# NVlabs/FoundationPose

Hardware: NVIDIA H100
Metric: pose-hypotheses/sec at 640x480 RGB-D, 252 hyp, 5 refine iters (higher is better)
Workload: dtype f16

## Files before the change

foundationpose_b200/csrc/fp_common.cuh:

```cuda
#pragma once
#include <cuda.h>
#include <cuda_fp16.h>
#include <cuda_runtime.h>
#include <stdint.h>
#include <stdio.h>
#include <string.h>

#include <atomic>

namespace fp {

void note_launches(int n);
unsigned long long launch_count();
void set_capturing(bool on);
inline bool device_bit_test(const std::atomic<unsigned long long>& m) {
  int d = 0;
  cudaGetDevice(&d);
  return (m.load(std::memory_order_acquire) >> (d & 63)) & 1ull;
}
inline void device_bit_set(std::atomic<unsigned long long>& m) {
  int d = 0;
  cudaGetDevice(&d);
  m.fetch_or(1ull << (d & 63), std::memory_order_release);
}
int num_sms();

void set_last_error(const char* fmt, ...);
int check_device_ptr(const void* p, const char* what, const char* fn = "fp_pose_errors");
#define FP_CUDA_OK(expr)                                                                   \
  do {                                                                                     \
    cudaError_t _e = (expr);                                                               \
    if (_e != cudaSuccess) {                                                               \
      fp::set_last_error("%s:%d: %s -> %s", __FILE__, __LINE__, #expr, cudaGetErrorString(_e)); \
      return -2;                                                                           \
    }                                                                                      \
  } while (0)
#define FP_REQUIRE(cond, ...)                                                              \
  do {                                                                                     \
    if (!(cond)) {                                                                         \
      fp::set_last_error(__VA_ARGS__);                                                     \
      return -1;                                                                           \
    }                                                                                      \
  } while (0)
#define FP_TRY(expr)     \
  do {                   \
    int _rc = (expr);    \
    if (_rc) return _rc; \
  } while (0)

bool pdl_enabled();
void pdl_skip_next();

template <typename... KArgs, typename... Args>
inline cudaError_t launch_pdl(void (*kernel)(KArgs...), dim3 grid, dim3 block, size_t smem, cudaStream_t stream,
                              int cluster_x, Args... args) {
  cudaLaunchConfig_t cfg;
  memset(&cfg, 0, sizeof(cfg));
  cfg.gridDim = grid;
  cfg.blockDim = block;
  cfg.dynamicSmemBytes = smem;
  cfg.stream = stream;
  cudaLaunchAttribute attr[2];
  int na = 0;
  if (cluster_x > 1) {
    attr[na].id = cudaLaunchAttributeClusterDimension;
    attr[na].val.clusterDim.x = cluster_x;
    attr[na].val.clusterDim.y = 1;
    attr[na].val.clusterDim.z = 1;
    ++na;
  }
  if (pdl_enabled()) {
    attr[na].id = cudaLaunchAttributeProgrammaticStreamSerialization;
    attr[na].val.programmaticStreamSerializationAllowed = 1;
    ++na;
  }
  cfg.attrs = attr;
  cfg.numAttrs = na;
  return cudaLaunchKernelEx(&cfg, kernel, KArgs(args)...);
}

__device__ __forceinline__ void pdl_wait() { asm volatile("griddepcontrol.wait;" ::: "memory"); }
__device__ __forceinline__ void pdl_trigger() { asm volatile("griddepcontrol.launch_dependents;" ::: "memory"); }

__device__ __forceinline__ uint32_t smem_u32(const void* p) {
  return static_cast<uint32_t>(__cvta_generic_to_shared(p));
}

__device__ __forceinline__ void mbar_init(uint64_t* bar, uint32_t count) {
  asm volatile("mbarrier.init.shared::cta.b64 [%0], %1;" ::"r"(smem_u32(bar)), "r"(count));
}
__device__ __forceinline__ void mbar_fence_init() {
  asm volatile("fence.mbarrier_init.release.cluster;" ::: "memory");
}
__device__ __forceinline__ void mbar_expect_tx(uint64_t* bar, uint32_t bytes) {
  asm volatile("mbarrier.arrive.expect_tx.shared::cta.b64 _, [%0], %1;" ::"r"(smem_u32(bar)),
               "r"(bytes)
               : "memory");
}
__device__ __forceinline__ void mbar_arrive(uint64_t* bar) {
  asm volatile("mbarrier.arrive.shared::cta.b64 _, [%0];" ::"r"(smem_u32(bar)) : "memory");
}
__device__ __forceinline__ void mbar_wait(uint64_t* bar, uint32_t parity) {
  asm volatile(
      "{\n\t"
      ".reg .pred P1;\n\t"
      "WAIT_%=:\n\t"
      "mbarrier.try_wait.parity.shared::cta.b64 P1, [%0], %1, %2;\n\t"
      "@P1 bra DONE_%=;\n\t"
      "bra WAIT_%=;\n\t"
      "DONE_%=:\n\t"
      "}" ::"r"(smem_u32(bar)),
      "r"(parity), "r"(0x989680)
      : "memory");
}

__device__ __forceinline__ void tma_load_5d(const CUtensorMap* map, uint64_t* bar, void* dst,
                                            int c0, int c1, int c2, int c3, int c4) {
  asm volatile(
      "cp.async.bulk.tensor.5d.shared::cluster.global.mbarrier::complete_tx::bytes"
      " [%0], [%1, {%3, %4, %5, %6, %7}], [%2];" ::"r"(smem_u32(dst)),
      "l"(reinterpret_cast<uint64_t>(map)), "r"(smem_u32(bar)), "r"(c0), "r"(c1), "r"(c2),
      "r"(c3), "r"(c4)
      : "memory");
}
__device__ __forceinline__ void tma_load_2d(const CUtensorMap* map, uint64_t* bar, void* dst,
                                            int c0, int c1) {
  asm volatile(
      "cp.async.bulk.tensor.2d.shared::cluster.global.mbarrier::complete_tx::bytes"
      " [%0], [%1, {%3, %4}], [%2];" ::"r"(smem_u32(dst)),
      "l"(reinterpret_cast<uint64_t>(map)), "r"(smem_u32(bar)), "r"(c0), "r"(c1)
      : "memory");
}
__device__ __forceinline__ void tma_store_5d(const CUtensorMap* map, const void* src, int c0, int c1, int c2, int c3,
                                             int c4) {
  asm volatile("cp.async.bulk.tensor.5d.global.shared::cta.bulk_group [%0, {%2, %3, %4, %5, %6}], [%1];" ::"l"(
                   reinterpret_cast<uint64_t>(map)),
               "r"(smem_u32(src)), "r"(c0), "r"(c1), "r"(c2), "r"(c3), "r"(c4)
               : "memory");
}
__device__ __forceinline__ void tma_prefetch_desc(const CUtensorMap* map) {
  asm volatile("prefetch.tensormap [%0];" ::"l"(reinterpret_cast<uint64_t>(map)) : "memory");
}

__device__ __forceinline__ uint32_t cluster_nctarank() {
  uint32_t r;
  asm volatile("mov.u32 %0, %%cluster_nctarank;" : "=r"(r));
  return r;
}
__device__ __forceinline__ uint32_t cluster_ctarank() {
  uint32_t r;
  asm volatile("mov.u32 %0, %%cluster_ctarank;" : "=r"(r));
  return r;
}
__device__ __forceinline__ void cluster_sync_all() {
  asm volatile("barrier.cluster.arrive.release.aligned;" ::: "memory");
  asm volatile("barrier.cluster.wait.acquire.aligned;" ::: "memory");
}

template <uint32_t N>
__device__ __forceinline__ void regs_release() {
  asm volatile("setmaxnreg.dec.sync.aligned.u32 %0;" ::"n"(N));
}
template <uint32_t N>
__device__ __forceinline__ void regs_acquire() {
  asm volatile("setmaxnreg.inc.sync.aligned.u32 %0;" ::"n"(N));
}

__device__ __forceinline__ void wgmma_fence() { asm volatile("wgmma.fence.sync.aligned;" ::: "memory"); }
__device__ __forceinline__ void wgmma_commit() { asm volatile("wgmma.commit_group.sync.aligned;" ::: "memory"); }
template <int N>
__device__ __forceinline__ void wgmma_wait() {
  asm volatile("wgmma.wait_group.sync.aligned %0;" ::"n"(N) : "memory");
}
template <int N>
__device__ __forceinline__ void fence_regs(float (&d)[N]) {
#pragma unroll
  for (int i = 0; i < N; ++i) asm volatile("" : "+f"(d[i])::"memory");
}

__device__ __forceinline__ uint64_t gmma_desc_sw128(uint32_t smem_addr, uint32_t sbo = 1024) {
  uint64_t d = 0;
  d |= (uint64_t)((smem_addr & 0x3FFFF) >> 4);
  d |= (uint64_t)1 << 16;
  d |= (uint64_t)(sbo >> 4) << 32;
  d |= (uint64_t)1 << 62;
  return d;
}
__device__ __forceinline__ uint64_t gmma_desc_mn_sw128(uint32_t smem_addr, uint32_t lbo) {
  uint64_t d = 0;
  d |= (uint64_t)((smem_addr & 0x3FFFF) >> 4);
  d |= (uint64_t)((lbo >> 4) & 0x3FFF) << 16;
  d |= (uint64_t)(1024 >> 4) << 32;
  d |= (uint64_t)1 << 62;
  return d;
}
__device__ __forceinline__ uint64_t gmma_desc_linear(uint32_t smem_addr, uint32_t lbo, uint32_t sbo) {
  uint64_t d = 0;
  d |= (uint64_t)((smem_addr & 0x3FFFF) >> 4);
  d |= (uint64_t)(lbo >> 4) << 16;
  d |= (uint64_t)(sbo >> 4) << 32;
  return d;
}

__device__ __forceinline__ void ldsm_x4_trans(uint32_t addr, uint32_t (&r)[4]) {
  asm volatile("ldmatrix.sync.aligned.m8n8.x4.trans.shared.b16 {%0, %1, %2, %3}, [%4];"
               : "=r"(r[0]), "=r"(r[1]), "=r"(r[2]), "=r"(r[3])
               : "r"(addr)
               : "memory");
}
__device__ __forceinline__ void stsm_x4_trans(uint32_t addr, const uint32_t (&r)[4]) {
  asm volatile("stmatrix.sync.aligned.m8n8.x4.trans.shared.b16 [%0], {%1, %2, %3, %4};" ::"r"(addr), "r"(r[0]),
               "r"(r[1]), "r"(r[2]), "r"(r[3])
               : "memory");
}

__device__ __forceinline__ uint32_t pack_half2(float a, float b) {
  __half2 h = __floats2half2_rn(a, b);
  return *reinterpret_cast<uint32_t*>(&h);
}

}
```

foundationpose_b200/csrc/fp_linear.cu:

```cuda
#include <stdlib.h>
#include <string.h>

#include "fp_common.cuh"
#include "fp_gemm.cuh"
#include "fp_wgmma.cuh"

namespace fp {

int encode_map_f16(CUtensorMap* map, const void* base, int rank, const uint64_t* dims, const uint64_t* strides_bytes,
                   const uint32_t* box);

constexpr int kLwsK = 512;
constexpr int kLwsKBlocks = kLwsK / 64;
constexpr int kLwsRows = 64;
constexpr int kLwsCols = 128;
constexpr int kLwsThreads = 384;
constexpr int kLwsBoxBytes = kLwsCols * 64 * 2;
constexpr int kLwsPanelBytes = kLwsKBlocks * kLwsBoxBytes;
constexpr int kLwsStages = kLwsKBlocks;
constexpr int kLwsStageBytes = kLwsRows * 64 * 2;
constexpr int kLwsSlabBytes = kLwsRows * 64 * 2;
constexpr int kLwsSlabs = 4;
constexpr int kLwsSmemBytes =
    kLwsPanelBytes + kLwsStages * kLwsStageBytes + kLwsSlabs * kLwsSlabBytes + 1024  + 256 ;
static_assert(kLwsSmemBytes <= 232448, "the weight-stationary linear kernel exceeds the 227 KB opt-in shared memory");
static_assert((2 * kLwsStages + 4) * 8 <= 256, "the mbarriers must fit their 256 bytes");

constexpr uint32_t kOrderBar = 2;
constexpr uint32_t kWgBar = 4;

struct LinearWsParams {
  int row_tiles;
  int total;
  const float* bias;
  int has_res;
  int relu;
};

__device__ __forceinline__ void named_sync(uint32_t id, uint32_t count) {
  asm volatile("bar.sync %0, %1;" ::"r"(id), "r"(count) : "memory");
}
__device__ __forceinline__ void named_arrive(uint32_t id, uint32_t count) {
  asm volatile("bar.arrive %0, %1;" ::"r"(id), "r"(count) : "memory");
}

__global__ void __launch_bounds__(kLwsThreads, 1)
    linear_ws_kernel(const __grid_constant__ CUtensorMap map_a, const __grid_constant__ CUtensorMap map_w,
                     const __grid_constant__ CUtensorMap map_out, const __grid_constant__ CUtensorMap map_res,
                     const __grid_constant__ LinearWsParams p) {
  extern __shared__ uint8_t smem_raw[];
  uint8_t* smem = smem_raw + ((1024u - (smem_u32(smem_raw) & 1023u)) & 1023u);
  uint8_t* panel = smem;
  uint8_t* ring = panel + kLwsPanelBytes;
  uint8_t* staging = ring + kLwsStages * kLwsStageBytes;
  uint64_t* bars = reinterpret_cast<uint64_t*>(staging + kLwsSlabs * kLwsSlabBytes);
  uint64_t* full = bars;
  uint64_t* empty = bars + kLwsStages;
  uint64_t* panel_full = bars + 2 * kLwsStages;
  uint64_t* panel_empty = panel_full + 1;
  uint64_t* res_full = panel_full + 2;

  const int i0 = (int)((long long)blockIdx.x * p.total / gridDim.x);
  const int n = (int)((long long)(blockIdx.x + 1) * p.total / gridDim.x) - i0;
  const int panel0 = i0 / p.row_tiles;
  const int jb = min(n, (panel0 + 1) * p.row_tiles - i0);
  const bool reload = jb < n;

  if (threadIdx.x == 0) {
    tma_prefetch_desc(&map_a);
    tma_prefetch_desc(&map_w);
    tma_prefetch_desc(&map_out);
    if (p.has_res) tma_prefetch_desc(&map_res);
    for (int s = 0; s < kLwsStages; ++s) {
      mbar_init(&full[s], 1);
      mbar_init(&empty[s], 128);
    }
    mbar_init(panel_full, 1);
    mbar_init(panel_empty, 256);
    mbar_init(&res_full[0], 1);
    mbar_init(&res_full[1], 1);
    mbar_fence_init();
    mbar_expect_tx(panel_full, kLwsPanelBytes);
    for (int kb = 0; kb < kLwsKBlocks; ++kb)
      tma_load_2d(&map_w, panel_full, panel + kb * kLwsBoxBytes, kb * 64, panel0 * kLwsCols);
  }
  __syncthreads();
  pdl_trigger();
  pdl_wait();

  if (threadIdx.x < 128) {
    if (threadIdx.x == 0) {
      for (int j = 0; j < n; ++j) {
        if (j == jb) {
          mbar_wait(panel_empty, 0);
          mbar_expect_tx(panel_full, kLwsPanelBytes);
          for (int kb = 0; kb < kLwsKBlocks; ++kb)
            tma_load_2d(&map_w, panel_full, panel + kb * kLwsBoxBytes, kb * 64, (panel0 + 1) * kLwsCols);
        }
        const int row0 = ((i0 + j) % p.row_tiles) * kLwsRows;
        for (int kb = 0; kb < kLwsKBlocks; ++kb) {
          mbar_wait(&empty[kb], (uint32_t)((j & 1) ^ 1));
          mbar_expect_tx(&full[kb], kLwsStageBytes);
          tma_load_2d(&map_a, &full[kb], ring + kb * kLwsStageBytes, kb * 64, row0);
        }
      }
    }
    return;
  }

  const int ct = threadIdx.x - 128;
  const int w = ct >> 7;
  const int lane = threadIdx.x & 31;
  const int r0 = 16 * ((ct >> 5) & 3) + (lane >> 2);
  const int cq = 2 * (lane & 3);
  const bool leader = (ct & 127) == 0;
  uint8_t* slabs = staging + w * 2 * kLwsSlabBytes;
  if (reload && w >= jb) mbar_arrive(panel_empty);
  float acc[64];
#pragma unroll
  for (int i = 0; i < 64; ++i) acc[i] = 0.f;
  for (int j = w, it = 0; j < n; j += 2, ++it) {
    const int item = i0 + j;
    const int pn = item / p.row_tiles;
    const int row0 = (item - pn * p.row_tiles) * kLwsRows;
    if (j > 0) named_sync(kOrderBar + w, 256);
    mbar_wait(panel_full, j >= jb ? 1u : 0u);
    for (int kb = 0; kb < kLwsKBlocks; ++kb) {
      mbar_wait(&full[kb], (uint32_t)(j & 1));
      const uint64_t da = gmma_desc_sw128(smem_u32(ring + kb * kLwsStageBytes));
      const uint64_t db = gmma_desc_sw128(smem_u32(panel + kb * kLwsBoxBytes));
      wgmma_fence();
#pragma unroll
      for (int k = 0; k < 4; ++k)
        Wgmma<128>::ss(acc, da + (uint64_t)(2 * k), db + (uint64_t)(2 * k), (kb > 0 || k > 0) ? 1u : 0u);
      wgmma_commit();
      if (kb == 0 && leader) {
        asm volatile("cp.async.bulk.wait_group.read 0;" ::: "memory");
        if (p.has_res) {
          mbar_expect_tx(&res_full[w], 2 * kLwsSlabBytes);
          for (int s = 0; s < 2; ++s)
            tma_load_5d(&map_res, &res_full[w], slabs + s * kLwsSlabBytes, pn * kLwsCols + 64 * s, row0, 0, 0, 0);
        }
      }
      if (kb > 0) {
        wgmma_wait<1>();
        mbar_arrive(&empty[kb - 1]);
      }
    }
    if (j + 1 < n) named_arrive(kOrderBar + (w ^ 1), 256);
    wgmma_wait<0>();
    fence_regs(acc);
    mbar_arrive(&empty[kLwsKBlocks - 1]);
    if (reload && j < jb && j + 2 >= jb) mbar_arrive(panel_empty);

    const float* bias = p.bias + pn * kLwsCols;
    if (p.has_res) mbar_wait(&res_full[w], (uint32_t)(it & 1));
    else named_sync(kWgBar + w, 128);
#pragma unroll
    for (int b = 0; b < 2; ++b) {
      uint8_t* slab = slabs + b * kLwsSlabBytes;
#pragma unroll
      for (int jh = 0; jh < 8; jh += 4) {
        float2 bb[4];
        __half2 rv[4][2];
#pragma unroll
        for (int jl = 0; jl < 4; ++jl) {
          bb[jl] = __ldg(reinterpret_cast<const float2*>(bias + 64 * b + 8 * (jh + jl) + cq));
          if (p.has_res) {
#pragma unroll
            for (int h = 0; h < 2; ++h) {
              const int row = r0 + 8 * h;
              rv[jl][h] = *reinterpret_cast<const __half2*>(slab + row * 128 + (((uint32_t)(jh + jl) ^ (uint32_t)(row & 7)) << 4) + cq * 2);
            }
          }
        }
#pragma unroll
        for (int jl = 0; jl < 4; ++jl) {
          const int jc = 8 * b + jh + jl;
#pragma unroll
          for (int h = 0; h < 2; ++h) {
            const int row = r0 + 8 * h;
            uint32_t* cell = reinterpret_cast<uint32_t*>(slab + row * 128 + (((uint32_t)(jh + jl) ^ (uint32_t)(row & 7)) << 4) + cq * 2);
            float a0 = acc[4 * jc + 2 * h] + bb[jl].x, a1 = acc[4 * jc + 2 * h + 1] + bb[jl].y;
            if (p.has_res) {
              const float2 r = __half22float2(rv[jl][h]);
              a0 += r.x;
              a1 += r.y;
            }
            if (p.relu) {
              a0 = fmaxf(a0, 0.f);
              a1 = fmaxf(a1, 0.f);
            }
            *cell = pack_half2(a0, a1);
          }
        }
      }
    }
    asm volatile("fence.proxy.async.shared::cta;" ::: "memory");
    named_sync(kWgBar + w, 128);
    if (leader) {
      for (int s = 0; s < 2; ++s)
        tma_store_5d(&map_out, slabs + s * kLwsSlabBytes, pn * kLwsCols + 64 * s, row0, 0, 0, 0);
      asm volatile("cp.async.bulk.commit_group;" ::: "memory");
    }
  }
  if (leader) asm volatile("cp.async.bulk.wait_group 0;" ::: "memory");
}

static bool linear_ws_enabled() {
  const char* e = getenv("FPOSE_LINEAR_WS");
  return !(e && e[0] == '0');
}

constexpr int kLinearWsMinItemsPerCta = 8;

bool linear_ws_takes(const GemmLayer& L) {
  if (L.kind != LK_LINEAR || L.Cin != kLwsK || L.Cout % kLwsCols != 0 || L.out_split != 0 || L.post_add ||
      !linear_ws_enabled())
    return false;
  const int sms = num_sms();
  const int panels = L.Cout / kLwsCols;
  const long long items = (long long)panels * ((L.Win + kLwsRows - 1) / kLwsRows);
  return sms > 0 && panels <= sms && items >= (long long)kLinearWsMinItemsPerCta * sms;
}

int linear_ws_launch(const GemmLayer& L, cudaStream_t stream) {
  const uint64_t E = 2;
  const int M = L.Win;
  LinearWsParams p;
  memset(&p, 0, sizeof(p));
  p.row_tiles = (M + kLwsRows - 1) / kLwsRows;
  p.total = (L.Cout / kLwsCols) * p.row_tiles;
  p.bias = L.bias;
  p.has_res = L.res != nullptr;
  p.relu = L.relu;
  CUtensorMap ma, mw, mo, mr;
  {
    const uint64_t d[2] = {(uint64_t)kLwsK, (uint64_t)M}, s[1] = {(uint64_t)kLwsK * E};
    const uint32_t b[2] = {64, kLwsRows};
    if (int rc = encode_map_f16(&ma, L.in, 2, d, s, b)) return rc;
  }
  {
    const uint64_t d[2] = {(uint64_t)kLwsK, (uint64_t)L.Cout}, s[1] = {(uint64_t)kLwsK * E};
    const uint32_t b[2] = {64, kLwsCols};
    if (int rc = encode_map_f16(&mw, L.w, 2, d, s, b)) return rc;
  }
  auto rows_map = [&](CUtensorMap* m, const void* base, int ld) {
    const uint64_t row = (uint64_t)ld * E;
    const uint64_t d[5] = {(uint64_t)ld, (uint64_t)M, 1, 1, 1}, s[4] = {row, row * M, row * M, row * M};
    const uint32_t b[5] = {64, kLwsRows, 1, 1, 1};
    return encode_map_f16(m, base, 5, d, s, b);
  };
  if (int rc = rows_map(&mo, L.out, L.out_ld)) return rc;
  mr = mo;
  if (L.res) {
    if (int rc = rows_map(&mr, L.res, L.res_ld)) return rc;
  }

  static std::atomic<unsigned long long> attr_mask{0};
  if (!device_bit_test(attr_mask)) {
    FP_CUDA_OK(cudaFuncSetAttribute(linear_ws_kernel, cudaFuncAttributeMaxDynamicSharedMemorySize, kLwsSmemBytes));
    device_bit_set(attr_mask);
  }
  const int sms = num_sms();
  FP_REQUIRE(sms > 0, "no CUDA device");
  const int grid = p.total < sms ? p.total : sms;
  prof_mark_begin(0, 2.0 * (double)M * L.Cout * kLwsK, stream);
  FP_CUDA_OK(launch_pdl(linear_ws_kernel, dim3(grid), dim3(kLwsThreads), kLwsSmemBytes, stream, 1, ma, mw, mo, mr, p));
  prof_mark_end(stream);
  note_launches(1);
  FP_CUDA_OK(cudaGetLastError());
  return 0;
}

}
```

foundationpose_b200/csrc/fp_stem.cu:

```cuda
#include <stdlib.h>
#include <string.h>

#include "fp_common.cuh"
#include "fp_gemm.cuh"
#include "fp_wgmma.cuh"

namespace fp {

int encode_map_f16(CUtensorMap* map, const void* base, int rank, const uint64_t* dims, const uint64_t* strides_bytes,
                   const uint32_t* box);
int encode_map_f16_linear(CUtensorMap* map, const void* base, int rank, const uint64_t* dims,
                          const uint64_t* strides_bytes, const uint32_t* box);
int num_sms();

namespace {

constexpr int kThreadsStem = 384;
constexpr int kTileH = 16, kTileW = 8;
constexpr int kPatchRows = 2 * (kTileH - 1) + 7;
constexpr int kPatchPairs = kTileW + 3;
constexpr int kParStride = kPatchPairs * 16;
constexpr int kRowStride = 2 * kParStride;
constexpr int kPatchBytes = kPatchRows * kRowStride;
constexpr int kPatchSlot = 13 * 1024;
constexpr int kStagesStem = 6;
constexpr int kWTileBytes = 2 * 64 * 16;
constexpr int kWBytes = 28 * kWTileBytes;
constexpr int kHalfSlab = 64 * 64 * 2;
constexpr int kStemSmem = kWBytes + kStagesStem * kPatchSlot + 4 * kHalfSlab + 1024 + 256;

struct StemParams {
  int tiles_w, tiles_h, n_img, total_tiles;
  const float* bias;
  int relu;
};

__device__ __forceinline__ void bulk_load_1d(void* dst, const void* src, uint32_t bytes, uint64_t* bar) {
  asm volatile("cp.async.bulk.shared::cluster.global.mbarrier::complete_tx::bytes [%0], [%1], %2, [%3];" ::"r"(
                   smem_u32(dst)),
               "l"(src), "r"(bytes), "r"(smem_u32(bar))
               : "memory");
}

__global__ void __launch_bounds__(kThreadsStem, 1)
    stem_conv_kernel(const __grid_constant__ CUtensorMap map_in, const __grid_constant__ CUtensorMap map_out,
                     const __half* __restrict__ wpack, const StemParams p) {
  constexpr int S = kStagesStem;
  extern __shared__ uint8_t smem_raw[];
  uint8_t* smem = reinterpret_cast<uint8_t*>((reinterpret_cast<uintptr_t>(smem_raw) + 1023) & ~uintptr_t(1023));
  uint8_t* wsm = smem;
  uint8_t* ring = smem + kWBytes;
  uint8_t* staging = ring + S * kPatchSlot;
  uint64_t* bars = reinterpret_cast<uint64_t*>(staging + 4 * kHalfSlab);
  uint64_t* full = bars;
  uint64_t* empty = bars + S;
  uint64_t* w_full = bars + 2 * S;

  if (threadIdx.x == 0) {
    tma_prefetch_desc(&map_in);
    tma_prefetch_desc(&map_out);
    for (int s = 0; s < S; ++s) {
      mbar_init(&full[s], 1);
      mbar_init(&empty[s], 256);
    }
    mbar_init(w_full, 1);
    mbar_fence_init();
  }
  __syncthreads();
  const int tiles_per_img = p.tiles_w * p.tiles_h;
  pdl_trigger();

  if (threadIdx.x < 128) {
    if (threadIdx.x == 0) {
      mbar_expect_tx(w_full, kWBytes);
      bulk_load_1d(wsm, wpack, kWBytes, w_full);
      pdl_wait();
      int stage = 0, phase = 0;
      for (int t = blockIdx.x; t < p.total_tiles; t += gridDim.x) {
        const int n = t / tiles_per_img, rem = t - n * tiles_per_img;
        const int th = rem / p.tiles_w, tw = rem - th * p.tiles_w;
        mbar_wait(&empty[stage], phase ^ 1);
        mbar_expect_tx(&full[stage], kPatchBytes);
        tma_load_5d(&map_in, &full[stage], ring + stage * kPatchSlot, tw * kTileW * 8, 0, th * 2 * kTileH, n, 0);
        if (++stage == S) {
          stage = 0;
          phase ^= 1;
        }
      }
    }
    return;
  }

  const int ct = threadIdx.x - 128;
  const int cw = ct >> 7;
  const int lane = threadIdx.x & 31;
  const int r0 = 16 * ((ct >> 5) & 3) + (lane >> 2);
  const int cq = 2 * (lane & 3);
  const bool leader = ((ct & 127) == 0);
  const uint32_t w_addr = smem_u32(wsm);
  float2 bias[8];
#pragma unroll
  for (int j = 0; j < 8; ++j) bias[j] = __ldg(reinterpret_cast<const float2*>(p.bias + 8 * j + cq));
  float acc[32];
#pragma unroll
  for (int i = 0; i < 32; ++i) acc[i] = 0.f;
  mbar_wait(w_full, 0);
  pdl_wait();
  int stage = 0, phase = 0, use = 0;
  for (int t = blockIdx.x; t < p.total_tiles; t += gridDim.x, ++use) {
    const int n = t / tiles_per_img, rem = t - n * tiles_per_img;
    const int th = rem / p.tiles_w, tw = rem - th * p.tiles_w;
    mbar_wait(&full[stage], phase);
    const uint32_t patch = smem_u32(ring + stage * kPatchSlot) + (uint32_t)(cw * 8 * 2 * kRowStride);
    wgmma_fence();
#pragma unroll
    for (int r = 0; r < 7; ++r) {
#pragma unroll
      for (int s = 0; s < 4; ++s) {
        const uint64_t da = gmma_desc_linear(patch + r * kRowStride + s * 16, kParStride, 2 * kRowStride);
        const uint64_t db = gmma_desc_linear(w_addr + (r * 4 + s) * kWTileBytes, 1024, 128);
        Wgmma<64>::ss(acc, da, db, (r | s) ? 1u : 0u);
      }
    }
    wgmma_commit();
    wgmma_wait<0>();
    fence_regs(acc);
    mbar_arrive(&empty[stage]);
    if (++stage == S) {
      stage = 0;
      phase ^= 1;
    }

    uint8_t* slab = staging + (cw * 2 + (use & 1)) * kHalfSlab;
    if (leader) asm volatile("cp.async.bulk.wait_group.read 1;" ::: "memory");
    asm volatile("bar.sync %0, 128;" ::"r"(1 + cw) : "memory");
#pragma unroll
    for (int j = 0; j < 8; ++j) {
#pragma unroll
      for (int h = 0; h < 2; ++h) {
        const int row = r0 + 8 * h;
        float a0 = acc[4 * j + 2 * h] + bias[j].x, a1 = acc[4 * j + 2 * h + 1] + bias[j].y;
        if (p.relu) {
          a0 = fmaxf(a0, 0.f);
          a1 = fmaxf(a1, 0.f);
        }
        *reinterpret_cast<uint32_t*>(slab + row * 128 + (((uint32_t)j ^ (uint32_t)(row & 7)) << 4) + cq * 2) =
            pack_half2(a0, a1);
      }
    }
    asm volatile("fence.proxy.async.shared::cta;" ::: "memory");
    asm volatile("bar.sync %0, 128;" ::"r"(1 + cw) : "memory");
    if (leader) {
      tma_store_5d(&map_out, slab, 0, tw * kTileW, th * kTileH + 8 * cw, n, 0);
      asm volatile("cp.async.bulk.commit_group;" ::: "memory");
    }
  }
  if (leader) asm volatile("cp.async.bulk.wait_group 0;" ::: "memory");
}

}

int stem_conv_launch(const GemmLayer& L, cudaStream_t stream) {
  FP_REQUIRE(L.Cin == 8 && L.Cout == 64, "CONV7_S2: the stem kernel is 8 (6 + 2 zero) -> 64 channels");
  FP_REQUIRE(L.Hin % (2 * kTileH) == 0 && L.Win % (2 * kTileW) == 0, "CONV7_S2: unsupported size %dx%d", L.Hin, L.Win);
  FP_REQUIRE(!L.res && !L.post_add && L.out_split == 0, "CONV7_S2: residual / post-add / split are not supported");
  FP_REQUIRE(L.out_ld % 8 == 0 && L.out_ld >= 64, "CONV7_S2: bad out_ld %d", L.out_ld);
  FP_REQUIRE((reinterpret_cast<uintptr_t>(L.w) & 15) == 0, "CONV7_S2: weights must be 16-byte aligned");
  if (L.n_img == 0) return 0;
  const int Ho = L.Hin / 2, Wo = L.Win / 2;
  const uint64_t E = 2;
  const uint64_t rows = L.Hin + 6, pairs = (L.Win + 8) / 2;
  CUtensorMap mi, mo;
  {
    uint64_t d[5] = {8 * pairs, 2, rows, (uint64_t)L.n_img, 1};
    uint64_t s[4] = {pairs * 8 * E, 2 * pairs * 8 * E, rows * 2 * pairs * 8 * E, rows * 2 * pairs * 8 * E * L.n_img};
    uint32_t b[5] = {8 * (uint32_t)kPatchPairs, 2, (uint32_t)kPatchRows, 1, 1};
    int rc = encode_map_f16_linear(&mi, L.in, 5, d, s, b);
    if (rc) return rc;
  }
  {
    uint64_t d[5] = {(uint64_t)L.out_ld, (uint64_t)Wo, (uint64_t)Ho, (uint64_t)L.n_img, 1};
    uint64_t s[4] = {(uint64_t)L.out_ld * E, (uint64_t)L.out_ld * E * Wo, (uint64_t)L.out_ld * E * Wo * Ho,
                     (uint64_t)L.out_ld * E * Wo * Ho * L.n_img};
    uint32_t b[5] = {64, (uint32_t)kTileW, (uint32_t)kTileH / 2, 1, 1};
    int rc = encode_map_f16(&mo, L.out, 5, d, s, b);
    if (rc) return rc;
  }
  StemParams p;
  p.tiles_w = Wo / kTileW;
  p.tiles_h = Ho / kTileH;
  p.n_img = L.n_img;
  p.total_tiles = p.tiles_w * p.tiles_h * L.n_img;
  p.bias = L.bias;
  p.relu = L.relu;
  static std::atomic<unsigned long long> attr_mask{0};
  if (!device_bit_test(attr_mask)) {
    FP_CUDA_OK(cudaFuncSetAttribute(stem_conv_kernel, cudaFuncAttributeMaxDynamicSharedMemorySize, kStemSmem));
    device_bit_set(attr_mask);
  }
  const int sms = num_sms();
  FP_REQUIRE(sms > 0, "no CUDA device");
  const int grid = p.total_tiles < sms ? p.total_tiles : sms;
  prof_mark_begin(0, 2.0 * (double)L.n_img * Ho * Wo * 64.0 * (7.0 * 7.0 * 6.0), stream);
  FP_CUDA_OK(launch_pdl(stem_conv_kernel, dim3(grid), dim3(kThreadsStem), kStemSmem, stream, 1, mi, mo,
                        reinterpret_cast<const __half*>(L.w), p));
  prof_mark_end(stream);
  note_launches(1);
  FP_CUDA_OK(cudaGetLastError());
  return 0;
}

}
```

Measured before the change: 3958.

## Ping-pong stem conv warpgroups over whole tiles and store epilogue via stmatrix

The stem conv kernel no longer splits each tile's rows across the two consumer warpgroups. Each warpgroup now owns alternate tiles and ring stages, computes both row halves with two accumulators, and passes an ordering barrier to the other warpgroup so one warpgroup's MMA can overlap the other's epilogue. The epilogue writes the swizzled staging slab with stmatrix x4 instead of scalar 32-bit shared stores, and one full-tile TMA store replaces two half stores. The cost is double the accumulator registers, larger staging slabs in shared memory, and more complex barrier and parity logic.

```diff
diff --git a/foundationpose_b200/csrc/fp_common.cuh b/foundationpose_b200/csrc/fp_common.cuh
--- a/foundationpose_b200/csrc/fp_common.cuh
+++ b/foundationpose_b200/csrc/fp_common.cuh
@@ -213,6 +213,18 @@
                "r"(r[1]), "r"(r[2]), "r"(r[3])
                : "memory");
 }
+__device__ __forceinline__ void stsm_x4(uint32_t addr, const uint32_t (&r)[4]) {
+  asm volatile("stmatrix.sync.aligned.m8n8.x4.shared.b16 [%0], {%1, %2, %3, %4};" ::"r"(addr), "r"(r[0]), "r"(r[1]),
+               "r"(r[2]), "r"(r[3])
+               : "memory");
+}
+
+__device__ __forceinline__ void named_sync(uint32_t id, uint32_t count) {
+  asm volatile("bar.sync %0, %1;" ::"r"(id), "r"(count) : "memory");
+}
+__device__ __forceinline__ void named_arrive(uint32_t id, uint32_t count) {
+  asm volatile("bar.arrive %0, %1;" ::"r"(id), "r"(count) : "memory");
+}
 
 __device__ __forceinline__ uint32_t pack_half2(float a, float b) {
   __half2 h = __floats2half2_rn(a, b);
diff --git a/foundationpose_b200/csrc/fp_linear.cu b/foundationpose_b200/csrc/fp_linear.cu
--- a/foundationpose_b200/csrc/fp_linear.cu
+++ b/foundationpose_b200/csrc/fp_linear.cu
@@ -37,13 +37,6 @@
   int relu;
 };
 
-__device__ __forceinline__ void named_sync(uint32_t id, uint32_t count) {
-  asm volatile("bar.sync %0, %1;" ::"r"(id), "r"(count) : "memory");
-}
-__device__ __forceinline__ void named_arrive(uint32_t id, uint32_t count) {
-  asm volatile("bar.arrive %0, %1;" ::"r"(id), "r"(count) : "memory");
-}
-
 __global__ void __launch_bounds__(kLwsThreads, 1)
     linear_ws_kernel(const __grid_constant__ CUtensorMap map_a, const __grid_constant__ CUtensorMap map_w,
                      const __grid_constant__ CUtensorMap map_out, const __grid_constant__ CUtensorMap map_res,
diff --git a/foundationpose_b200/csrc/fp_stem.cu b/foundationpose_b200/csrc/fp_stem.cu
--- a/foundationpose_b200/csrc/fp_stem.cu
+++ b/foundationpose_b200/csrc/fp_stem.cu
@@ -26,8 +26,13 @@
 constexpr int kStagesStem = 6;
 constexpr int kWTileBytes = 2 * 64 * 16;
 constexpr int kWBytes = 28 * kWTileBytes;
-constexpr int kHalfSlab = 64 * 64 * 2;
-constexpr int kStemSmem = kWBytes + kStagesStem * kPatchSlot + 4 * kHalfSlab + 1024 + 256;
+constexpr int kSlab = kTileH * kTileW * 64 * 2;
+constexpr int kStemSmem = kWBytes + kStagesStem * kPatchSlot + 4 * kSlab + 1024 + 256;
+static_assert(kStagesStem % 2 == 0, "each warpgroup must own the ring stages of its parity");
+static_assert(kStemSmem <= 232448, "the stem kernel exceeds the 227 KB opt-in shared memory");
+
+constexpr uint32_t kOrderBar = 1;
+constexpr uint32_t kWgBar = 3;
 
 struct StemParams {
   int tiles_w, tiles_h, n_img, total_tiles;
@@ -51,7 +56,7 @@
   uint8_t* wsm = smem;
   uint8_t* ring = smem + kWBytes;
   uint8_t* staging = ring + S * kPatchSlot;
-  uint64_t* bars = reinterpret_cast<uint64_t*>(staging + 4 * kHalfSlab);
+  uint64_t* bars = reinterpret_cast<uint64_t*>(staging + 4 * kSlab);
   uint64_t* full = bars;
   uint64_t* empty = bars + S;
   uint64_t* w_full = bars + 2 * S;
@@ -61,7 +66,7 @@
     tma_prefetch_desc(&map_out);
     for (int s = 0; s < S; ++s) {
       mbar_init(&full[s], 1);
-      mbar_init(&empty[s], 256);
+      mbar_init(&empty[s], 128);
     }
     mbar_init(w_full, 1);
     mbar_fence_init();
@@ -92,66 +97,79 @@
   }
 
   const int ct = threadIdx.x - 128;
-  const int cw = ct >> 7;
+  const int w = ct >> 7;
   const int lane = threadIdx.x & 31;
-  const int r0 = 16 * ((ct >> 5) & 3) + (lane >> 2);
   const int cq = 2 * (lane & 3);
+  const int sm_row = 16 * ((ct >> 5) & 3) + 8 * ((lane >> 3) & 1) + (lane & 7);
+  const uint32_t sm_chunk = (uint32_t)(lane >> 4);
   const bool leader = ((ct & 127) == 0);
   const uint32_t w_addr = smem_u32(wsm);
+  const uint32_t slabs = smem_u32(staging + w * 2 * kSlab);
   float2 bias[8];
 #pragma unroll
   for (int j = 0; j < 8; ++j) bias[j] = __ldg(reinterpret_cast<const float2*>(p.bias + 8 * j + cq));
-  float acc[32];
-#pragma unroll
-  for (int i = 0; i < 32; ++i) acc[i] = 0.f;
+  float acc[2][32];
+#pragma unroll
+  for (int h = 0; h < 2; ++h)
+#pragma unroll
+    for (int k = 0; k < 32; ++k) acc[h][k] = 0.f;
   mbar_wait(w_full, 0);
   pdl_wait();
-  int stage = 0, phase = 0, use = 0;
-  for (int t = blockIdx.x; t < p.total_tiles; t += gridDim.x, ++use) {
+  int use = 0;
+  for (int i = w, t = blockIdx.x + w * gridDim.x; t < p.total_tiles; i += 2, t += 2 * gridDim.x, ++use) {
     const int n = t / tiles_per_img, rem = t - n * tiles_per_img;
     const int th = rem / p.tiles_w, tw = rem - th * p.tiles_w;
-    mbar_wait(&full[stage], phase);
-    const uint32_t patch = smem_u32(ring + stage * kPatchSlot) + (uint32_t)(cw * 8 * 2 * kRowStride);
+    const int stage = i % S;
+    if (i > 0) named_sync(kOrderBar + w, 256);
+    mbar_wait(&full[stage], (uint32_t)((i / S) & 1));
+    const uint32_t patch = smem_u32(ring + stage * kPatchSlot);
     wgmma_fence();
 #pragma unroll
     for (int r = 0; r < 7; ++r) {
 #pragma unroll
       for (int s = 0; s < 4; ++s) {
-        const uint64_t da = gmma_desc_linear(patch + r * kRowStride + s * 16, kParStride, 2 * kRowStride);
         const uint64_t db = gmma_desc_linear(w_addr + (r * 4 + s) * kWTileBytes, 1024, 128);
-        Wgmma<64>::ss(acc, da, db, (r | s) ? 1u : 0u);
+#pragma unroll
+        for (int h = 0; h < 2; ++h) {
+          const uint64_t da =
+              gmma_desc_linear(patch + h * 8 * 2 * kRowStride + r * kRowStride + s * 16, kParStride, 2 * kRowStride);
+          Wgmma<64>::ss(acc[h], da, db, (r | s) ? 1u : 0u);
+        }
       }
     }
     wgmma_commit();
+    if (t + gridDim.x < p.total_tiles) named_arrive(kOrderBar + (w ^ 1), 256);
+    if (leader) asm volatile("cp.async.bulk.wait_group.read 1;" ::: "memory");
     wgmma_wait<0>();
-    fence_regs(acc);
+    fence_regs(acc[0]);
+    fence_regs(acc[1]);
     mbar_arrive(&empty[stage]);
-    if (++stage == S) {
-      stage = 0;
-      phase ^= 1;
-    }
-
-    uint8_t* slab = staging + (cw * 2 + (use & 1)) * kHalfSlab;
-    if (leader) asm volatile("cp.async.bulk.wait_group.read 1;" ::: "memory");
-    asm volatile("bar.sync %0, 128;" ::"r"(1 + cw) : "memory");
-#pragma unroll
-    for (int j = 0; j < 8; ++j) {
-#pragma unroll
-      for (int h = 0; h < 2; ++h) {
-        const int row = r0 + 8 * h;
-        float a0 = acc[4 * j + 2 * h] + bias[j].x, a1 = acc[4 * j + 2 * h + 1] + bias[j].y;
-        if (p.relu) {
-          a0 = fmaxf(a0, 0.f);
-          a1 = fmaxf(a1, 0.f);
+
+    const uint32_t slab = slabs + (use & 1) * kSlab;
+    named_sync(kWgBar + w, 128);
+#pragma unroll
+    for (int h = 0; h < 2; ++h) {
+#pragma unroll
+      for (int q = 0; q < 4; ++q) {
+        uint32_t v[4];
+#pragma unroll
+        for (int m = 0; m < 4; ++m) {
+          const int j = 2 * q + (m >> 1), e = 2 * (m & 1);
+          float a0 = acc[h][4 * j + e] + bias[j].x, a1 = acc[h][4 * j + e + 1] + bias[j].y;
+          if (p.relu) {
+            a0 = fmaxf(a0, 0.f);
+            a1 = fmaxf(a1, 0.f);
+          }
+          v[m] = pack_half2(a0, a1);
         }
-        *reinterpret_cast<uint32_t*>(slab + row * 128 + (((uint32_t)j ^ (uint32_t)(row & 7)) << 4) + cq * 2) =
-            pack_half2(a0, a1);
+        const int row = 64 * h + sm_row;
+        stsm_x4(slab + row * 128 + (((2 * q + sm_chunk) ^ (uint32_t)(row & 7)) << 4), v);
       }
     }
     asm volatile("fence.proxy.async.shared::cta;" ::: "memory");
-    asm volatile("bar.sync %0, 128;" ::"r"(1 + cw) : "memory");
+    named_sync(kWgBar + w, 128);
     if (leader) {
-      tma_store_5d(&map_out, slab, 0, tw * kTileW, th * kTileH + 8 * cw, n, 0);
+      tma_store_5d(&map_out, staging + (w * 2 + (use & 1)) * kSlab, 0, tw * kTileW, th * kTileH, n, 0);
       asm volatile("cp.async.bulk.commit_group;" ::: "memory");
     }
   }
@@ -182,7 +200,7 @@
     uint64_t d[5] = {(uint64_t)L.out_ld, (uint64_t)Wo, (uint64_t)Ho, (uint64_t)L.n_img, 1};
     uint64_t s[4] = {(uint64_t)L.out_ld * E, (uint64_t)L.out_ld * E * Wo, (uint64_t)L.out_ld * E * Wo * Ho,
                      (uint64_t)L.out_ld * E * Wo * Ho * L.n_img};
-    uint32_t b[5] = {64, (uint32_t)kTileW, (uint32_t)kTileH / 2, 1, 1};
+    uint32_t b[5] = {64, (uint32_t)kTileW, (uint32_t)kTileH, 1, 1};
     int rc = encode_map_f16(&mo, L.out, 5, d, s, b);
     if (rc) return rc;
   }
```

After: 3984 (median of 6 runs). No clear change (+0.6%).
